# Zhehui-Huang/quad-swarm-rl

Hardware: AMD Instinct MI355X
Metric: env-steps/s (drones x envs x sim_steps) (higher is better)
Workload: dtype f32

## Files before the change

### __graft_entry__.py

```python
import os
import subprocess
import sys

REPO = os.path.dirname(os.path.abspath(__file__))
if REPO not in sys.path:
    sys.path.insert(0, REPO)


def build():
    from quad_swarm_rl_amd import native
    native.build(force=True, verbose=True)
    assert os.path.exists(native.LIB_PATH)
    from quad_swarm_rl_amd import policy
    policy.build(force=True, verbose=True)
    assert os.path.exists(policy.ENC_LIB_PATH)
    subprocess.check_call(["make", "-C", os.path.join(REPO, "oracle"), "-s", "-B"])
    import quad_swarm_rl_amd
    from quad_swarm_rl_amd import config, env
    import ctypes
    lib = ctypes.CDLL(native.LIB_PATH)
    for sym in native.EXPORTED_SYMBOLS + native.EXCHANGE_SYMBOLS:
        getattr(lib, sym)
    paths = prebuild_spec_cache()
    print(f"build ok: {native.LIB_PATH} + {len(paths)} config-specialised code objects in spec_cache/")


def _spec_jobs(with_audit=True):
    import bench
    jobs = []
    for wl in bench.WORKLOADS.values():
        for rew_info in (False, True):
            jobs.append((dict(wl["kw"], num_envs=wl["num_envs"], write_rew_info=rew_info), "f32"))
        jobs.append((dict(wl["kw"], num_envs=wl["num_envs"]), "f64"))
        jobs.append((dict(wl["kw"], num_envs=wl["num_envs"], write_rew_info=False), "f32", 0))
        jobs.append((dict(wl["kw"], num_envs=wl["num_envs"], write_rew_info=False, episode_sums=True), "f32"))
        jobs.append((dict(wl["kw"], num_envs=wl["num_envs"], write_rew_info=True, episode_sums=True), "f32"))
        jobs.append((dict(wl["kw"], num_envs=wl["num_envs"], write_rew_info=False, use_downwash=False), "f32"))
        if not wl["kw"].get("use_obstacles"):
            jobs.append((dict(wl["kw"], num_envs=wl["num_envs"], write_rew_info=False, episode_sums=True, quads_mode="mix"), "f32"))
    smoke_kw = dict(num_envs=4, num_agents=8, neighbor_visible_num=6, neighbor_obs_type="pos_vel", use_downwash=True, use_numba=True,
                    collision_falloff_radius=4.0, rew_coeff=dict(quadcol_bin=5.0, quadcol_bin_smooth_max=10.0))
    jobs += [(smoke_kw, "f64"), (smoke_kw, "f32"), (dict(smoke_kw, write_rew_info=False), "f32")]
    try:
        sys.path.insert(0, os.path.join(REPO, "tests"))
        import test_hip_parity as thp
        for kw in thp.CASES.values():
            jobs += [(dict(kw, num_envs=8), "f64"), (dict(kw, num_envs=8), "f32")]
        for name in ("c2_n8_dw", "c3_n8_obst", "c4_n32_svs"):
            jobs += [(dict(thp.CASES[name], num_envs=512, ep_time=0.3), "f32"), (dict(thp.CASES[name], num_envs=40, ep_time=0.5), "f32"),
                     (dict(thp.CASES[name], num_envs=40, ep_time=0.5), "f64")]
        for name, E in (("c2_n8_dw", 1024), ("c3_n8_obst", 1024), ("c4_n32_svs", 512)):
            jobs.append((dict(thp.CASES[name], num_envs=E, ep_time=0.3), "f64"))
        for name in ("c2_n8_dw", "c4_n32_svs"):
            jobs.append((dict(thp.CASES[name], num_envs=96, ep_time=0.3), "f32"))
        for name in thp.SINGLE_WAVE_CASES:
            jobs += [(dict(thp.CASES[name], num_envs=8), "f64", 0), (dict(thp.CASES[name], num_envs=8), "f32", 0)]
        import test_object_identity_gpu as toi
        for name in toi.POISON_CASES:
            for team in (0, 1):
                kw = dict(thp.CASES[name], num_envs=7, **toi.POISON_OVERRIDES.get(name, {}))
                prec = "f32" if team and kw["num_agents"] > 8 else "f64"
                jobs.append((kw, prec, team))
                jobs += [(kw, prec, team, {"QS_SPEC_EXTRA_FLAGS": f"-DQS_POISON_IDLE={m}"}) for m in (1, 2)]
        for name in toi.SCHED_SINGLE:
            jobs += [(dict(thp.CASES[name], num_envs=7), "f32", 0), (dict(thp.CASES[name], num_envs=7), "f32", 0, {"QS_SPEC_SINGLE_FLAGS": "-mllvm -amdgpu-use-amdgpu-trackers"})]
        for name in ("c2_n8_dw", "c3_n8_obst", "c4_n32_svs"):
            jobs += [(dict(thp.CASES[name], num_envs=7), "f32", 1), (dict(thp.CASES[name], num_envs=7), "f32", 1, {"QS_SPEC_TEAM_FLAGS": ""})]
        for name in toi.RESPONSE_CASES:
            for prec in ("f64", "f32"):
                if prec == "f64" and thp.CASES[name]["num_agents"] > 8:
                    continue
                jobs += [(dict(thp.CASES[name], num_envs=7), prec, 1), (dict(thp.CASES[name], num_envs=7), prec, 1, {"QS_SPEC_EXTRA_FLAGS": "-DQS_SERIAL_PAIR_RESPONSES"})]
        for name in toi.SELECT_CASES:
            jobs += [(dict(thp.CASES[name], num_envs=7), "f32", 0)] + [(dict(thp.CASES[name], num_envs=7), "f32", 0, {"QS_SPEC_EXTRA_FLAGS": f})
                                                                       for f in ("-DQS_EXACT_NBR_SELECT", "-DQS_NBR_TRUNC_BITS=16")]
        for name in toi.STASH_CASES:
            jobs += [(dict(thp.CASES[name], num_envs=7), "f32", 1), (dict(thp.CASES[name], num_envs=7), "f32", 1, {"QS_SPEC_EXTRA_FLAGS": "-DQS_SN_STASH=0"})]
        for name in toi.REDO_CASES:
            jobs += [(dict(thp.CASES[name], num_envs=7), "f32", 1), (dict(thp.CASES[name], num_envs=7), "f32", 1, {"QS_SPEC_EXTRA_FLAGS": "-DQS_REDO_ROWS=0"})]
        import xchg_worker as xw
        jobs += [(dict(xw.KW, num_envs=8, write_rew_info=False), "f32"), (dict(xw.KW, num_envs=4, episode_sums=True), "f32"),
                 (dict(xw.REPLAY_KW, num_envs=8, write_rew_info=False, episode_sums=True), "f32")]
        import test_pilot_gpu as tpg
        jobs.append((dict(tpg.LOOP_KW, num_envs=1024), "f32"))
    except Exception as exc:
        print("spec prebuild: parity cases skipped:", exc)
    finally:
        sys.path.pop(0)
    if with_audit:
        jobs += _audit_jobs()
    return jobs


def _audit_jobs():
    import base64
    import ctypes
    import json
    from quad_swarm_rl_amd import config as qcfg
    path = os.path.join(REPO, "tests", "spec_audit.json")
    if not os.path.exists(path):
        return []
    doc = json.load(open(path))
    if doc.get("sizeof_qs_config") != ctypes.sizeof(qcfg.QsConfig):
        print("spec prebuild: tests/spec_audit.json was written for another qs_config layout - rerun tools/spec_audit.py; skipped")
        return []
    return [(base64.b64decode(o["config"]), None, o["team"]) for o in doc["objects"]]


def _spec_one(job):
    from quad_swarm_rl_amd import config as qcfg, native
    kw, precision = job[0], job[1]
    team = job[2] if len(job) > 2 else -1
    build_env = job[3] if len(job) > 3 else {}
    saved = {k: os.environ.get(k) for k in build_env}
    os.environ.update(build_env)
    try:
        cfg = qcfg.QsConfig.from_buffer_copy(kw) if isinstance(kw, bytes) else qcfg.make_config(precision=precision, **kw)
        return native.spec_build(cfg, team)
    except native.QsError as exc:
        print("spec prebuild skipped:", exc)
        return None
    finally:
        for k, v in saved.items():
            if v is None:
                os.environ.pop(k, None)
            else:
                os.environ[k] = v


def prebuild_spec_cache():
    from concurrent.futures import ProcessPoolExecutor
    jobs = _spec_jobs()
    with ProcessPoolExecutor(max_workers=min(8, os.cpu_count() or 1)) as ex:
        paths = sorted(set(p for p in ex.map(_spec_one, jobs) if p))
    if not paths:
        return paths
    keep = {os.path.splitext(os.path.basename(p))[0] for p in paths}
    cache = os.path.dirname(paths[0])
    for f in os.listdir(cache):
        if os.path.splitext(f)[0] not in keep:
            os.remove(os.path.join(cache, f))
    return paths


def smoke():
    import numpy as np
    from oracle import oracle as orc
    from quad_swarm_rl_amd import config as qcfg, native

    def worst(got, ref, tol, omega_cols=False, relative=False):
        allowed = np.full(ref.shape, tol)
        if relative:
            allowed = tol * np.maximum(1.0, np.abs(ref))
        elif omega_cols:
            allowed[..., 15:18] = tol * np.maximum(1.0, np.abs(ref[..., 15:18]))
        return float((np.abs(got - ref) / allowed).max())

    E, N = 4, 8
    for precision, tol in (("f64", 1e-8), ("f32", 1e-5)):
        cfg = qcfg.make_config(num_envs=E, num_agents=N, neighbor_visible_num=6, neighbor_obs_type="pos_vel",
                               use_downwash=True, use_numba=True, collision_falloff_radius=4.0, seed=11, precision=precision,
                               rew_coeff=dict(quadcol_bin=5.0, quadcol_bin_smooth_max=10.0))
        hip = native.Stepper(cfg, device=0)
        oenvs = [orc.OracleEnv(cfg, env_global_id=e) for e in range(E)]
        oobs = np.stack([o.reset() for o in oenvs])
        hip.reset()
        hobs = hip.to_host("obs").reshape(E, N, -1)
        assert worst(hobs, oobs, tol, omega_cols=True) <= 1.0, (precision, "reset", worst(hobs, oobs, tol, omega_cols=True))
        rng = np.random.RandomState(0)
        for t in range(3):
            act = rng.uniform(-1, 1, size=(E, N, 4)).astype(np.float32).astype(np.float64)
            o = [oe.step(act[e]) for e, oe in enumerate(oenvs)]
            hip.from_host("actions", act.reshape(-1, 4))
            hip.step()
            hip.sync()
            hobs = hip.to_host("obs").reshape(E, N, -1)
            hrew = hip.to_host("reward").reshape(E, N)
            err = max(worst(hobs, np.stack([x[0] for x in o]), tol, omega_cols=True), worst(hrew, np.stack([x[1] for x in o]), tol, relative=True))
            assert err <= 1.0, (precision, t, err)
        hip.check_errors()
        hip.close()
        print(f"smoke {precision}: ok (every observation column within {tol} absolute; angular velocity and reward within {tol} * max(1, |x|))")


if __name__ == "__main__":
    build()
    if len(sys.argv) > 1 and sys.argv[1] == "smoke":
        smoke()
```

### quad-swarm-rl_amd/csrc/qs_nbr_obs.h

```cpp
#pragma once
#include "qs_device.h"

using namespace qs;

__device__ __forceinline__ unsigned long long nbr_key(float m, int idx) {
    const uint32_t b = __float_as_uint(m), o = b ^ ((b >> 31) ? 0xffffffffu : 0x80000000u);
    return ((unsigned long long)o << 32) | (uint32_t)idx;
}

template <typename real> __device__ __forceinline__ real nbr_metric(const real rp[3], const real rv[3]) {
    const real rd = M<real>::fmax(norm3<real>(rp), (real)0.01);
    return rd + (rp[0] * rv[0] + rp[1] * rv[1] + rp[2] * rv[2]) * M<real>::rcp(rd);
}
template <> __device__ __forceinline__ float nbr_metric<float>(const float rp[3], const float rv[3]) {
    const float d2 = __builtin_fmaf(rp[2], rp[2], __builtin_fmaf(rp[1], rp[1], rp[0] * rp[0]));
    const float dot = __builtin_fmaf(rp[2], rv[2], __builtin_fmaf(rp[1], rv[1], rp[0] * rv[0]));
    const float rd = fmaxf(__builtin_amdgcn_sqrtf(d2), 0.01f);
    return __builtin_fmaf(dot, __builtin_amdgcn_rcpf(rd), rd);
}
typedef float qs_f32x2 __attribute__((ext_vector_type(2)));
__device__ __forceinline__ qs_f32x2 nbr_metric_x2(const qs_f32x2 rp[3], const qs_f32x2 rv[3]) {
    const qs_f32x2 d2 = __builtin_elementwise_fma(rp[2], rp[2], __builtin_elementwise_fma(rp[1], rp[1], rp[0] * rp[0]));
    const qs_f32x2 dot = __builtin_elementwise_fma(rp[2], rv[2], __builtin_elementwise_fma(rp[1], rv[1], rp[0] * rv[0]));
    const qs_f32x2 rd = {fmaxf(__builtin_amdgcn_sqrtf(d2.x), 0.01f), fmaxf(__builtin_amdgcn_sqrtf(d2.y), 0.01f)};
    const qs_f32x2 rc = {__builtin_amdgcn_rcpf(rd.x), __builtin_amdgcn_rcpf(rd.y)};
    return __builtin_elementwise_fma(dot, rc, rd);
}
template <typename real> struct NbrKey;
template <> struct NbrKey<float> {
    unsigned long long k;
    static __device__ __forceinline__ NbrKey make(float m, int j) { return {nbr_key(m, j)}; }
    __device__ __forceinline__ bool less(const NbrKey &o) const { return k < o.k; }
    __device__ __forceinline__ int idx() const { return (int)(uint32_t)k; }
    static __device__ __forceinline__ void st(unsigned char *base, int slots, int slot, int B, int tid,
        const NbrKey &v) { ((unsigned long long *)base)[slot * B + tid] = v.k; }
    static __device__ __forceinline__ NbrKey ld(const unsigned char *base, int slots, int slot, int B,
        int tid) { return {((const unsigned long long *)base)[slot * B + tid]}; }
};
template <> struct NbrKey<double> {
    double m; int j;
    static __device__ __forceinline__ NbrKey make(double m, int j) { return {m, j}; }
    __device__ __forceinline__ bool less(const NbrKey &o) const { return (m < o.m) | ((m == o.m) & (j < o.j)); }
    __device__ __forceinline__ int idx() const { return j; }
    static __device__ __forceinline__ void st(unsigned char *base, int slots, int slot, int B, int tid, const NbrKey &v) {
        ((double *)base)[slot * B + tid] = v.m; ((int *)(base + (size_t)slots * B * 8))[slot * B + tid] = v.j; }
    static __device__ __forceinline__ NbrKey ld(const unsigned char *base, int slots, int slot, int B, int tid) {
        return {((const double *)base)[slot * B + tid], ((const int *)(base + (size_t)slots * B * 8))[slot * B + tid]}; }
};

template <typename real>
__device__ __forceinline__ void neighbor_obs(const Consts<real> &c, int N, int i, int base, int B, int tid, const real *s_pos,
    const real *s_vel,
                                             real *s_metric, const real mypos[3], const real myvel[3], real *o) {
    const int K = c.num_neighbors;
    if (K <= 0) return;
    if (K == N - 1 || N <= 8) {
        const bool all_others = (K == N - 1);
        for (int j0 = 0; j0 < N; j0 += 8) {
            real rp[8][3], rv[8][3];
            int rank[8];
#pragma unroll
            for (int u = 0; u < 8; ++u) {
                const int j = (j0 + u < N) ? j0 + u : N - 1;
#pragma unroll
                for (int a = 0; a < 3; ++a) { rp[u][a] = s_pos[a * B + base + j] - mypos[a];
                    rv[u][a] = s_vel[a * B + base + j] - myvel[a]; }
            }
            if (all_others) {
#pragma unroll
                for (int u = 0; u < 8; ++u) rank[u] = (j0 + u < i) ? j0 + u : j0 + u - 1;
            } else {
                real mj[8];
#pragma unroll
                for (int u = 0; u < 8; ++u) {
                    real rd = M<real>::fmax(norm3<real>(rp[u]), (real)0.01);
                    real m = rd + (rp[u][0] * rv[u][0] + rp[u][1] * rv[u][1] + rp[u][2] * rv[u][2]) * M<real>::rcp(rd);
                    mj[u] = (u < N && u != i) ? m : (real)3.4e38;
                    rank[u] = 0;
                }
#pragma unroll
                for (int k = 0; k < 8; ++k)
#pragma unroll
                    for (int u = 0; u < 8; ++u) rank[u] += (int)((mj[k] < mj[u]) | ((mj[k] == mj[u]) & (k < u)));
            }
#pragma unroll
            for (int u = 0; u < 8; ++u) {
                const int j = j0 + u;
                if (j < N && j != i && rank[u] < K) {
                    real *oo = o + rank[u] * 6;
#pragma unroll
                    for (int a = 0; a < 3; ++a) {
                        oo[a] = clipr<real>(rp[u][a], -c.nbr_clip_pos[a], c.nbr_clip_pos[a]);
                        oo[3 + a] = clipr<real>(rv[u][a], -c.nbr_clip_vel[a], c.nbr_clip_vel[a]);
                    }
                }
            }
        }
        return;
    }
    if (K <= 8) {
        real bm[8];
        int bi[8];
#pragma unroll
        for (int k = 0; k < 8; ++k) { bm[k] = (real)3.4e38; bi[k] = 0; }
        for (int j0 = 0; j0 < N; j0 += 4) {
            real rp[4][3], rv[4][3];
#pragma unroll
            for (int u = 0; u < 4; ++u) {
                const int j = (j0 + u < N) ? j0 + u : N - 1;
#pragma unroll
                for (int a = 0; a < 3; ++a) { rp[u][a] = s_pos[a * B + base + j] - mypos[a];
                    rv[u][a] = s_vel[a * B + base + j] - myvel[a]; }
            }
#pragma unroll
            for (int u = 0; u < 4; ++u) {
                const int j = j0 + u;
                real rd = M<real>::fmax(norm3<real>(rp[u]), (real)0.01);
                real m = rd + (rp[u][0] * rv[u][0] + rp[u][1] * rv[u][1] + rp[u][2] * rv[u][2]) * M<real>::rcp(rd);
                m = (j < N && j != i) ? m : (real)3.4e38;
                int mi = j;
#pragma unroll
                for (int k = 0; k < 8; ++k) {
                    const bool lt = m < bm[k];
                    const real tm = lt ? bm[k] : m;
                    const int ti = lt ? bi[k] : mi;
                    bm[k] = lt ? m : bm[k];
                    bi[k] = lt ? mi : bi[k];
                    m = tm; mi = ti;
                }
            }
        }
        real vals[8][6];
#pragma unroll
        for (int k = 0; k < 8; ++k) {
            if (k < K) {
#pragma unroll
                for (int a = 0; a < 3; ++a) { vals[k][a] = s_pos[a * B + base + bi[k]] - mypos[a];
                    vals[k][3 + a] = s_vel[a * B + base + bi[k]] - myvel[a]; }
            }
        }
#pragma unroll
        for (int k = 0; k < 8; ++k) {
            if (k < K) {
#pragma unroll
                for (int a = 0; a < 3; ++a) {
                    o[k * 6 + a] = clipr<real>(vals[k][a], -c.nbr_clip_pos[a], c.nbr_clip_pos[a]);
                    o[k * 6 + 3 + a] = clipr<real>(vals[k][3 + a], -c.nbr_clip_vel[a], c.nbr_clip_vel[a]);
                }
            }
        }
        return;
    }
    for (int j = 0; j < N; ++j) {
        real rp[3] = {s_pos[0 * B + base + j] - mypos[0], s_pos[1 * B + base + j] - mypos[1], s_pos[2 * B + base + j] - mypos[2]};
        real rv[3] = {s_vel[0 * B + base + j] - myvel[0], s_vel[1 * B + base + j] - myvel[1], s_vel[2 * B + base + j] - myvel[2]};
        real rd = M<real>::fmax(norm3<real>(rp), (real)0.01);
        real mm = rd + (rp[0] * rv[0] + rp[1] * rv[1] + rp[2] * rv[2]) * M<real>::rcp(rd);
        s_metric[j * B + tid] = (j == i) ? (real)3.4e38 : mm;
    }
    uint64_t taken = 1ull << i;
    for (int k = 0; k < K; ++k) {
        int best = -1;
        real bmin = (real)3.4e38;
        for (int j = 0; j < N; ++j) {
            real mm = s_metric[j * B + tid];
            bool better = !(taken >> j & 1) && (best < 0 || mm < bmin);
            best = better ? j : best;
            bmin = better ? mm : bmin;
        }
        taken |= 1ull << best;
#pragma unroll
        for (int a = 0; a < 3; ++a) {
            o[k * 6 + a] = clipr<real>(s_pos[a * B + base + best] - mypos[a], -c.nbr_clip_pos[a], c.nbr_clip_pos[a]);
            o[k * 6 + 3 + a] = clipr<real>(s_vel[a * B + base + best] - myvel[a], -c.nbr_clip_vel[a], c.nbr_clip_vel[a]);
        }
    }
}

template <typename real> struct NbrSel {
// ... 244 lines not shown
```

### quad-swarm-rl_amd/csrc/qs_step_team.inc

```
#undef e_state_or_e
#if QS_MULTI
#define e_state_or_e e_state
#else
#define e_state_or_e e
#endif
#ifndef QS_GATED
#define QS_GATED 0
#endif
#ifdef QS_SPEC
#if QS_MULTI && QS_GATED
extern "C" __global__ void __launch_bounds__(64 * QS_TW) qs_spec_gated(QS_KARGS, int QS_EPB_ARG, int ksteps) {
#elif QS_MULTI
extern "C" __global__ void __launch_bounds__(64 * QS_TW) qs_spec_rollout(QS_KARGS, int QS_EPB_ARG, int ksteps) {
#else
extern "C" __global__ void __launch_bounds__(64 * QS_TW) qs_spec_step(QS_KARGS, int QS_EPB_ARG) {
    const int t = 0;
#endif
#else
template <typename real>
#if QS_MULTI && QS_GATED && QS_SCEN_FULL
__global__ void __launch_bounds__(64 * QS_TW) qs_gated_team_full(QS_KARGS, int QS_EPB_ARG, int ksteps) {
#elif QS_MULTI && QS_GATED
__global__ void __launch_bounds__(64 * QS_TW) qs_gated_team(QS_KARGS, int QS_EPB_ARG, int ksteps) {
#elif QS_MULTI && QS_SCEN_FULL
__global__ void __launch_bounds__(64 * QS_TW) qs_rollout_team_full(QS_KARGS, int QS_EPB_ARG, int ksteps) {
#elif QS_MULTI
__global__ void __launch_bounds__(64 * QS_TW) qs_rollout_team(QS_KARGS, int QS_EPB_ARG, int ksteps) {
#elif QS_SCEN_FULL
__global__ void __launch_bounds__(64 * QS_TW) qs_step_team_full(QS_KARGS, int QS_EPB_ARG) {
    const int t = 0;
#else
__global__ void __launch_bounds__(64 * QS_TW) qs_step_team(QS_KARGS, int QS_EPB_ARG) {
    const int t = 0;
#endif
#endif
    extern __shared__ __align__(16) unsigned char smem[];
    constexpr int W = QS_TW, WS = QS_TW - 1;
#ifndef QS_PAIR_ONCE
#define QS_PAIR_ONCE 1
#endif
    QS_SPEC_PROLOGUE
    const Consts<real> *cp = &c;
    real rewc[QS_REW_COUNT + 1];
#pragma unroll
    for (int q = 0; q <= QS_REW_COUNT; ++q) rewc[q] = p.rew_rt[q];
#define QS_OBST_SIZE (c.dr_on ? p.obst_size_env[ee] : c.obst_size)
    const int B = QS_WAVE, N = c.num_agents, E = c.num_envs, T = E * N, M_ = c.num_obstacles, K = c.num_neighbors;
    uint64_t *s_mask = (uint64_t *)(smem + L.off_mask);
    uint32_t *s_envflag = (uint32_t *)(smem + L.off_envflag);
    real *s_pos = (real *)(smem + L.off_pos), *s_vel = (real *)(smem + L.off_vel), *s_zax = (real *)(smem + L.off_zax);
    real *s_om = (real *)(smem + L.off_om), *s_goal = (real *)(smem + L.off_goal), *s_obs = (real *)(smem + L.off_obs);
    real *s_obst = (real *)(smem + L.off_obst), *s_metric = (real *)(smem + L.off_metric);
    real *s_rot6 = (real *)(smem + L.off_t_rot), *s_gpub = (real *)(smem + L.off_t_goal), *s_prox = (real *)(smem + L.off_t_prox);
    uint64_t *s_colm = (uint64_t *)(smem + L.off_t_col), *s_dwm = (uint64_t *)(smem + L.off_t_dw),
        *s_nearm = (uint64_t *)(smem + L.off_t_near);
    int *s_ohit = (int *)(smem + L.off_t_ohit);
    real *s_ri = (real *)(smem + L.off_t_ri);
    int *s_redo = (int *)(smem + L.off_t_redo);
    unsigned char *s_topk = smem + L.off_topk;
    const bool pair_once = QS_PAIR_ONCE && N > 8;
#ifndef QS_SN_STASH
#ifdef QS_SPEC
#define QS_SN_STASH 1
#else
#define QS_SN_STASH 0
#endif
#endif
#ifndef QS_REDO_ROWS
#ifdef QS_SPEC
#define QS_REDO_ROWS 1
#else
#define QS_REDO_ROWS 0
#endif
#endif

    QS_POISON_LDS(L.total, 64 * QS_TW);
    const int wv = __builtin_amdgcn_readfirstlane((int)(threadIdx.x >> 6));
    const int tid = threadIdx.x & 63, le = tid / N, i = tid - le * N, e = blockIdx.x * epb + le, base = le * N;
    const bool active = (le < epb) && (e < E);
    const int g = active ? e * N + i : 0, ee = active ? e : 0;
    const uint64_t nmask = (N >= 64) ? ~0ull : ((1ull << N) - 1);
    real *myobs = s_obs + tid * c.obs_dim;
    const __amdgpu_buffer_rsrc_t rs = QS_BUF_RSRC(p);
    QS_ROW(real, pos, rs, p, T, g); QS_ROW(real, vel, rs, p, T, g); QS_ROW(real, rot, rs, p, T, g); QS_ROW(real, omega, rs, p, T, g);
    QS_ROW(real, rot_damp, rs, p, T, g); QS_ROW(real, cmds_damp, rs, p, T, g); QS_ROW(real, ou, rs, p, T, g);
    QS_ROW(real, goal, rs, p, T, g);
    QS_ROW(real, ring, rs, p, T, g); QS_ROW(real, sums, rs, p, T, g); QS_ROW(uint32_t, flags, rs, p, T, g);
    QS_ROW(uint64_t, pair, rs, p, T, g);

    QS_STAMP(0);
    QS_STAMPW(0);
    QS_STAMP_WG(0);
    Drone<real> d;
    real goal[3], act[4], ring[4], sums[3];
    int32_t cnt[QS_CNT_COUNT];
    uint64_t prev_pair = 0;
    int tick_before = 0, svs_period = 0;
#if QS_SCEN_FULL && defined(QS_SPEC_N)
    ScenRegs<real> sreg;
#endif
    uint32_t step_no = 0;
    uint32_t step_raw = 0;
    if (wv <= 1 || (QS_SN_STASH && !QS_MULTI && wv == 2)) step_raw = p.step_ctr[ee];
    if (wv == 0) {
        if (b_pos.wide) {
            b_pos.template ldv<3>(d.pos); b_vel.template ldv<3>(d.vel); b_omega.template ldv<3>(d.omega); b_goal.template ldv<3>(goal);
            b_sums.template ldv<3>(sums);
            b_rot.template ldv<9>(d.rot);
            b_rot_damp.template ldv<4>(d.rot_damp); b_cmds_damp.template ldv<4>(d.cmds_damp); b_ou.template ldv<4>(d.ou);
            b_ring.template ldv<4>(ring);
        } else {
#pragma unroll
            for (int q = 0; q < 3; ++q) { d.pos[q] = b_pos.ld(q); d.vel[q] = b_vel.ld(q); d.omega[q] = b_omega.ld(q);
                goal[q] = b_goal.ld(q); sums[q] = b_sums.ld(q); }
#pragma unroll
            for (int q = 0; q < 9; ++q) d.rot[q] = b_rot.ld(q);
#pragma unroll
            for (int q = 0; q < 4; ++q) { d.rot_damp[q] = b_rot_damp.ld(q); d.cmds_damp[q] = b_cmds_damp.ld(q); d.ou[q] = b_ou.ld(q);
                ring[q] = b_ring.ld(q); }
        }
        d.flags = b_flags.ld();
        prev_pair = b_pair.ld();
        QS_POISON_DRONE(d); QS_POISON_ARR(goal, 3, 16); QS_POISON_ARR(sums, 3, 16); QS_POISON_ARR(ring, 4, 16); QS_POISON_U64(prev_pair);
        tick_before = p.tick[ee];
        svs_period = (c.scenario == QS_SCENARIO_SWARM_VS_SWARM) ? p.scen_int[ee] : 0;
        if (active && i == 0) {
#pragma unroll
            for (int q = 0; q < QS_CNT_COUNT; ++q) cnt[q] = p.counters[q * E + ee];
        }
#if QS_SCEN_FULL
#ifdef QS_SPEC_N
        if (active) scen_regs_load<real>(p, E, e, i, sreg);
#else
        if (active) scen_lds_load<real>(p, L, smem, E, e, le, i, N);
#endif
#endif
        asm volatile("" : "+v"(step_raw));
        step_no = step_raw + 1;
    } else if (wv == 1 || (QS_SN_STASH && !QS_MULTI && wv == 2)) {
        step_no = step_raw + 1;
    }
    if (wv == W - 1 && c.use_obstacles && active) {
        for (int k = i; k < M_; k += N) {
            s_obst[(le * 2 + 0) * M_ + k] = p.obst_pos[(size_t)e * M_ + k];
            s_obst[(le * 2 + 1) * M_ + k] = p.obst_pos[(size_t)E * M_ + (size_t)e * M_ + k];
        }
    }
#if QS_SCEN_FULL
    real *s_sr = (real *)(smem + L.off_sr) + le * SR_COUNT;
    int *s_si = (int *)(smem + L.off_si) + le * SI_COUNT;
#endif
    constexpr int WL = 2;
    const bool logw = (wv == WL) && active;
    real rsum[QS_SUM_COUNT];
    if (logw && c.episode_sums) {
#pragma unroll
        for (int q = 0; q < QS_SUM_COUNT; ++q) rsum[q] = p.run_sums[q * T + g];
    }
#if !QS_MULTI
    unsigned long long xq_seq = 0, xq_ack = ~0ull;
    if constexpr (sizeof(real) == 4) {
        if (p.xchg != nullptr) {
            xq_seq = p.xchg->loc->push_seq;
            if (wv == 0 && tid < p.xchg->world) xq_ack = qsx::ld_sys(&p.xchg->mine->ack[tid]);
        }
    }
#endif
    uint64_t out_curr_pair = 0;
    bool nan_any = false;
#if QS_MULTI
    const int g_state = g, e_state = e;
#if QS_GATED
    qsx::Gate *const G = (qsx::Gate *)p.xchg;
    const unsigned long long gseq0 = (unsigned long long)(uintptr_t)actions;
    bool gate_dead = false;
    unsigned long long *s_pre_seq = (unsigned long long *)s_ri;
    unsigned int *s_actpre = (unsigned int *)((char *)s_ri + 16);
    unsigned long long pf_flag = 0, pf_flag_next = 0;
    if (threadIdx.x == 0) *s_pre_seq = 0;
#endif
    for (int t = 0; t < ksteps; ++t) {
    int g = g_state, e = e_state;
    asm volatile("" : "+v"(g), "+v"(e));
#endif
    RngKey key = {c.seed_lo, c.seed_hi, (uint32_t)(c.env_id_offset + ee), step_no};
    SensNoise<real> sn;
    real rew = 0, ri[QS_RI_COUNT];
    bool nan_rew = false, done = false;
    int tick = 0;
#if QS_GATED
    bool pf_hold_issue = false;
    unsigned int pf_hold[sizeof(real)] = {};
#endif
    if (wv == 0) {
#if QS_GATED
        {
            const unsigned long long seq = gseq0 + (unsigned long long)t + 1;
            if (*s_pre_seq == seq) {
                if constexpr (sizeof(real) == 4) {
#pragma unroll
                    for (int q = 0; q < 4; ++q) act[q] = __uint_as_float(s_actpre[tid * 4 + q]);
                } else {
#pragma unroll
                    for (int q = 0; q < 4; ++q) act[q] = __longlong_as_double(((long long)s_actpre[tid * 8 + 2 * q + 1] << 32) | s_actpre[tid * 8 + 2 * q]);
                }
            } else {
            if (!gate_dead && !qsx::poll_ge_agent(&G->act_flag[blockIdx.x / G->wg_per_group], seq, G->timeout_ticks)) {
                gate_dead = true;
                if (tid == 0) atomicOr(&G->status, 1u);
            }
            const char *a = G->act_ring + ((seq - 1) % G->ring_len) * G->act_stride + (size_t)g * 4 * sizeof(real);
            if constexpr (sizeof(real) == 4) {
                const qsx::u32x4_t v = qsx::ld16_sc1(a);
                act[0] = __uint_as_float(v.x); act[1] = __uint_as_float(v.y); act[2] = __uint_as_float(v.z); act[3] = __uint_as_float(v.w);
            } else {
                const qsx::u32x4_t v0 = qsx::ld16_sc1(a), v1 = qsx::ld16_sc1(a + 16);
                act[0] = __longlong_as_double(((long long)v0.y << 32) | v0.x);
                act[1] = __longlong_as_double(((long long)v0.w << 32) | v0.z);
                act[2] = __longlong_as_double(((long long)v1.y << 32) | v1.x);
                act[3] = __longlong_as_double(((long long)v1.w << 32) | v1.z);
            }
            }
        }
#else
        {
            const real *a = actions + ((size_t)t * T + g) * 4;
#pragma unroll
// ... 150 lines not shown
    if (wv == 1) {
        QS_SELF_OBS_W1();
    } else if (active) {
        const int lane3 = (wv == 0) ? 0 : wv - 1;
        const real mp[3] = {s_pos[0 * B + tid], s_pos[1 * B + tid], s_pos[2 * B + tid]};
        const real pr = rewc[QS_REW_COUNT];
        uint32_t colm_lo = 0, colm_hi = 0, dwm_lo = 0, dwm_hi = 0;
        real prox = 0;
        for (int j0 = lane3; j0 < N; j0 += 2 * WS) {
            real rel[2][3], zx[2][3];
#pragma unroll
            for (int u = 0; u < 2; ++u) {
                const int j = (j0 + WS * u < N) ? j0 + WS * u : N - 1;
#pragma unroll
                for (int a = 0; a < 3; ++a) { rel[u][a] = mp[a] - s_pos[a * B + base + j]; zx[u][a] = s_zax[a * B + base + j]; }
            }
#pragma unroll
            for (int u = 0; u < 2; ++u) {
                const int j = j0 + WS * u;
                const bool other = (j < N) & (j != i);
                real dist = M<real>::sqrt(rel[u][0] * rel[u][0] + rel[u][1] * rel[u][1] + rel[u][2] * rel[u][2]);
                const uint32_t hit = (uint32_t)(other & (dist <= c.collision_threshold));
                prox += (other & (dist <= c.collision_falloff_threshold)) ? pr * dist + rewc[QS_REW_QUADCOL_SMOOTH_MAX] : (real)0;
                real rz = dot3<real>(rel[u], zx[u]), rxy = M<real>::sqrt(dist * dist - rz * rz);
                const uint32_t dw = (uint32_t)(other & ((real)-0.7 < rz) & (rz < (real)0) & (rxy < (real)0.1));
                if (N <= 32 || j < 32) { colm_lo |= hit << (j & 31); dwm_lo |= dw << (j & 31); }
                else { colm_hi |= hit << (j & 31); dwm_hi |= dw << (j & 31); }
            }
        }
        const uint64_t colm = colm_lo | ((uint64_t)colm_hi << 32), dwm = dwm_lo | ((uint64_t)dwm_hi << 32);
        if (colm) atomicOr((unsigned long long *)&s_colm[tid], (unsigned long long)colm);
        if (dwm) atomicOr((unsigned long long *)&s_dwm[tid], (unsigned long long)dwm);
        s_prox[lane3 * B + tid] = prox;
        if (wv == W - 1) {
            int obst_idx = -1;
            if (c.use_obstacles) {
                const real *ox = s_obst + (le * 2 + 0) * M_, *oy = s_obst + (le * 2 + 1) * M_;
                for (int k = M_ - 1; k >= 0; --k) {
                    real dx = mp[0] - ox[k], dy = mp[1] - oy[k];
                    obst_idx = (M<real>::sqrt(dx * dx + dy * dy) <= (c.dr_on
                        ? c.arm_r + (real)0.5 * QS_OBST_SIZE : c.obst_hit_threshold)) ? k : obst_idx;
                }
            }
            s_ohit[tid] = obst_idx;
        }
    }
    QS_STAMPW(3);
    QS_TEAM_BARRIER();
    QS_STAMP(6); QS_STAMP_WGK(8);
    QS_STAMPW(4);

    uint64_t curr_pair = 0, unique = 0, m_obst_new = 0, m_room = 0, new_pair = 0;
    bool refresh_obs = false;
    int obst_idx = -1;
    real eps_dist[3] = {0, 0, 0};
    if (wv == 0) {
        uint64_t dw_mask = 0;
        bool in_curr = false;
        real prox = 0;
        uint32_t bits = 0;
        if (active) {
            const uint64_t colm = s_colm[tid];
            in_curr = colm != 0;
            curr_pair = (i >= 63) ? 0 : (colm & ~((2ull << i) - 1));
            dw_mask = s_dwm[tid];
            if (pair_once) {
                uint64_t nm = s_nearm[tid];
                while (__builtin_expect(nm != 0, 0)) {
                    const int j = __ffsll((long long)nm) - 1;
                    nm &= nm - 1;
                    const real rel[3] = {d.pos[0] - s_pos[0 * B + base + j], d.pos[1] - s_pos[1 * B + base + j],
                        d.pos[2] - s_pos[2 * B + base + j]};
                    prox += rewc[QS_REW_COUNT] * M<real>::sqrt(rel[0] * rel[0] + rel[1] * rel[1] + rel[2] * rel[2]) + rewc[QS_REW_QUADCOL_SMOOTH_MAX];
                }
            } else {
                prox = s_prox[0 * B + tid];
#pragma unroll
                for (int q = 1; q < WS; ++q) prox += s_prox[q * B + tid];
            }
            if (c.use_obstacles) {
                obst_idx = s_ohit[tid];
                obstacle_hit_bits(obst_idx, d.flags, bits);
            }
            room_collision_bits(d.flags, bits);
        }
        new_pair = curr_pair & ~prev_pair;
        const EnvEvents ev = env_events<real>(c, active, in_curr, new_pair, bits, d.flags, base, nmask, i, tick, tick_before, myobs);
        unique = ev.unique; m_obst_new = ev.obst_new; m_room = ev.room;
        collision_rewards<real>(c, rewc, ev, i, bits, prox, rew, ri);
        if (c.write_rew_info || c.episode_sums) {
#pragma unroll
            for (int q = 0; q < QS_RI_COUNT; ++q) s_ri[q * B + tid] = ri[q];
            s_ri[QS_RI_COUNT * B + tid] = done ? (real)1 : (real)0;
        }
#if QS_SCEN_FULL
        goal_distance_log<real, false>(c, active ? s_sr[SR_METRIC] : (real)0, tick, done, d.flags, ring, sums, ri, eps_dist);
#else
        goal_distance_log<real, false>(c, c.approach_goal_metric, tick, done, d.flags, ring, sums, ri, eps_dist);
#endif
        if (active && i == 0) env_counters_add<real>(c, cnt, ev);

        QS_STAMP(7); QS_STAMP_WGK(9);
        const real vel_before[3] = {d.vel[0], d.vel[1], d.vel[2]};
        downwash_phase<real>(c, key, d, s_pos, s_zax, B, base, nmask, N, i, active, dw_mask, bits, (int *)nullptr,
            (const double *)nullptr, WaveSync());
        QS_STAMP(8);
        const bool any_dw = ((__ballot(active && (bits & B_DOWNWASH)) >> base) & nmask) != 0;
        static_assert((W - 1) * QS_WAVE >= QS_DD_CHUNK * QS_DD_DRAWS, "the draw table fits the proximity rows");
#ifdef QS_SERIAL_PAIR_RESPONSES
        pair_responses<real>(key, d, ev, new_pair, active, N, i, tid, base, B, s_pos, s_vel, s_om, s_mask, (int *)nullptr, WaveSync());
#else
        pair_responses<real>(key, d, ev, new_pair, active, N, i, tid, base, B, s_pos, s_vel, s_om, s_mask, (int *)nullptr, WaveSync(), s_prox);
#endif
        room_obstacle_phase<real>(cp, key, d, active, N, i, bits, obst_idx, s_obst + (le * 2 + 0) * M_, s_obst + (le * 2 + 1) * M_,
            p.obst_size_env + ee, (int *)nullptr, WaveSync());
        const bool update_flag = any_dw || (ev.newpair_any != 0) || (ev.obst_new != 0) || (ev.wall != 0) || (ev.ceil != 0);

#if QS_SCEN_FULL
        {
            ScenCtx<real> x = {s_sr, s_si, (uint64_t *)(smem + L.off_omap) + le * 4, s_goal + le * L.goal_rows * 3, s_zax, B, base, N};
            scenario_phase_full<real>(c, key, x, active, N, i, tick, goal, (int *)s_mask + base, (int *)nullptr, WaveSync());
        }
#else
        svs_phase<real>(c, p, key, active, N, E, e, i, tick, svs_period, s_goal + le * L.goal_rows * 3, (int *)s_mask + base, goal,
            (int *)nullptr, WaveSync());
#endif
        QS_STAMP(9); QS_STAMP_WGK(10);
#pragma unroll
        for (int q = 0; q < 3; ++q) s_vel[q * B + tid] = d.vel[q];
        refresh_obs = update_flag && active;
        if (pair_once) {
            const bool vel_changed = active && (bits_differ(d.vel[0], vel_before[0]) | bits_differ(d.vel[1], vel_before[1]) |
                bits_differ(d.vel[2], vel_before[2]));
            const uint32_t changed = (uint32_t)((__ballot(vel_changed) >> base) & nmask);
            if (active && i == 0) s_redo[le] = QS_REDO_ROWS && N <= 32 ? (int)changed : (update_flag ? 1 : 0);
        } else if (__builtin_expect(refresh_obs, 0)) {
            if (c.sense_noise) {
                if (stash_sn) {
                    const real *o = myobs + c.self_dim;
#pragma unroll
                    for (int q = 0; q < 3; ++q) { sn.p[q] = o[q]; sn.v[q] = o[3 + q]; sn.w[q] = o[6 + q]; sn.th[q] = o[9 + q]; }
                } else sensor_noise_draw<real>(c, key, i, 1, sn);
            }
            self_obs<real>(c, sn, d, goal, myobs);
        }
    } else if (pair_once) {
        if (wv == 1 && !c.use_obstacles) QS_SELF_OBS_W1();
        if (ranked && K <= 8 && active) team_rank_local<real, W>(N, i, base, B, tid, wv, s_pos, s_vel, s_metric, s_topk, false);
    }
    QS_STAMPW(5);
    QS_TEAM_BARRIER();
    QS_STAMP(14); QS_STAMP_WGK(11);
    QS_STAMPW(6);
    real mpos[3] = {0, 0, 0}, mvel[3] = {0, 0, 0};
    if (K > 0 && active) {
#pragma unroll
        for (int q = 0; q < 3; ++q) { mpos[q] = s_pos[q * B + tid]; mvel[q] = s_vel[q * B + tid]; }
    }
    const bool po_big = pair_once && K > 0 && K < N - 1 && K <= 8;
    const bool redo = pair_once && active && s_redo[le] != 0;
    if (QS_REDO_ROWS && N <= 32 && po_big) {
        bool wg_redo = false;
        for (int q = 0; q < epb; ++q) wg_redo |= s_redo[q] != 0;
        if (__builtin_expect(wg_redo, 0)) {
            if (wv >= 1) {
                uint32_t m = active ? (uint32_t)s_redo[le] : 0u;
                for (int idx = 0; __any(m != 0); ++idx) {
                    const int a = m ? __ffs((int)m) - 1 : -1;
                    m &= m - 1;
                    if (a >= 0 && a != i && idx % (W - 1) == wv - 1) {
                        const real rp[3] = {s_pos[0 * B + base + a] - mpos[0], s_pos[1 * B + base + a] - mpos[1], s_pos[2 * B + base + a] - mpos[2]};
                        const real rv[3] = {s_vel[0 * B + base + a] - mvel[0], s_vel[1 * B + base + a] - mvel[1], s_vel[2 * B + base + a] - mvel[2]};
                        const real mm = nbr_metric<real>(rp, rv);
                        s_metric[a * B + tid] = mm; s_metric[i * B + base + a] = mm;
                    }
                }
            }
            QS_TEAM_BARRIER();
            if (wv >= 1 && redo) team_rank_local<real, W>(N, i, base, B, tid, wv, s_pos, s_vel, s_metric, s_topk, false);
        }
    }
    if (pair_once && wv == 0 && __builtin_expect(refresh_obs, 0)) {
        if (c.sense_noise) {
            if (stash_sn) {
                const real *o = myobs + c.self_dim;
#pragma unroll
                for (int q = 0; q < 3; ++q) { sn.p[q] = o[q]; sn.v[q] = o[3 + q]; sn.w[q] = o[6 + q]; sn.th[q] = o[9 + q]; }
            } else sensor_noise_draw<real>(c, key, i, 1, sn);
        }
        self_obs<real>(c, sn, d, goal, myobs);
    }
    if (logw && (c.write_rew_info || c.episode_sums)) {
        real r[QS_RI_COUNT];
#pragma unroll
        for (int q = 0; q < QS_RI_COUNT; ++q) r[q] = s_ri[q * B + tid];
        const bool fin = s_ri[QS_RI_COUNT * B + tid] != (real)0;
        if (c.write_rew_info) {
#pragma unroll
            for (int q = 0; q < QS_RI_COUNT; ++q) p.rew_info[q * T + g] = r[q];
        }
        if (c.episode_sums) {
            real a4[4];
#if QS_GATED
            {
                const char *a = G->act_ring + ((gseq0 + (unsigned long long)t) % G->ring_len) * G->act_stride + (size_t)g * 4 * sizeof(real);
#pragma unroll
                for (int q = 0; q < 4; ++q) {
                    if constexpr (sizeof(real) == 4) a4[q] = __uint_as_float(qsx::ld4_sc1(a + 4 * q));
                    else a4[q] = __longlong_as_double(((long long)qsx::ld4_sc1(a + 8 * q + 4) << 32) | qsx::ld4_sc1(a + 8 * q));
                }
            }
#else
            {
                const real *a = actions + ((size_t)t * T + g) * 4;
#pragma unroll
                for (int q = 0; q < 4; ++q) a4[q] = a[q];
            }
#endif
#pragma unroll
            for (int q = 0; q < QS_SUM_COUNT; ++q) {
                const real add = q < QS_RI_COUNT
                    ? r[q < QS_RI_COUNT ? q : 0] : (q < QS_SUM_ACT2
                    ? a4[(q - QS_SUM_ACT) & 3] : a4[(q - QS_SUM_ACT2) & 3] * a4[(q - QS_SUM_ACT2) & 3]);
                const real v = rsum[q] + add;
                if (fin) p.ep_sums[q * T + g] = v;
                rsum[q] = fin ? (real)0 : v;
            }
        }
    }
#ifdef QS_EXP_NOBIG
    const bool big = false;
#else
    const bool big = !pair_once && N > 8 && K <= 8;
#endif
    real bm[8];
    int bi[8];
    int *s_mlist_i = (int *)(s_metric + W * 8 * B);
    if (QS_REDO_ROWS && N <= 32 && po_big) {
    } else
    if (po_big && wv >= 1 && __builtin_expect(redo, 0)) team_rank_local<real,
        W>(N, i, base, B, tid, wv, s_pos, s_vel, s_metric, s_topk, true);
    if (ranked && active && !big && !po_big && (!pair_once || redo)) {
        for (int j0 = wv; j0 < N; j0 += 2 * W) {
            real rp[2][3], rv[2][3];
#pragma unroll
            for (int u = 0; u < 2; ++u) {
                const int j = (j0 + W * u < N) ? j0 + W * u : N - 1;
#pragma unroll
                for (int a = 0; a < 3; ++a) { rp[u][a] = s_pos[a * B + base + j] - mpos[a]; rv[u][a] = s_vel[a * B + base + j] - mvel[a]; }
            }
#pragma unroll
            for (int u = 0; u < 2; ++u) {
                const int j = j0 + W * u;
                real rd = M<real>::fmax(norm3<real>(rp[u]), (real)0.01);
                real m = rd + (rp[u][0] * rv[u][0] + rp[u][1] * rv[u][1] + rp[u][2] * rv[u][2]) * M<real>::rcp(rd);
                if (j < N) s_metric[j * B + tid] = (j != i) ? m : (real)3.4e38;
            }
        }
    }
    if (ranked && active && big) {
#pragma unroll
        for (int k = 0; k < 8; ++k) { bm[k] = (real)3.4e38; bi[k] = 0x7fffffff; }
        for (int j0 = wv; j0 < N; j0 += 2 * W) {
            real rp[2][3], rv[2][3];
#pragma unroll
            for (int u = 0; u < 2; ++u) {
                const int j = (j0 + W * u < N) ? j0 + W * u : N - 1;
#pragma unroll
                for (int a = 0; a < 3; ++a) { rp[u][a] = s_pos[a * B + base + j] - mpos[a]; rv[u][a] = s_vel[a * B + base + j] - mvel[a]; }
            }
#pragma unroll
            for (int u = 0; u < 2; ++u) {
                const int j = j0 + W * u;
                real rd = M<real>::fmax(norm3<real>(rp[u]), (real)0.01);
                real m = rd + (rp[u][0] * rv[u][0] + rp[u][1] * rv[u][1] + rp[u][2] * rv[u][2]) * M<real>::rcp(rd);
                const bool valid = (j < N) & (j != i);
                m = valid ? m : (real)3.4e38;
                int mi = valid ? j : 0x7fffffff;
#pragma unroll
                for (int k = 0; k < 8; ++k) {
                    const bool lt = m < bm[k];
                    const real tm = lt ? bm[k] : m;
                    const int ti = lt ? bi[k] : mi;
                    bm[k] = lt ? m : bm[k];
                    bi[k] = lt ? mi : bi[k];
                    m = tm; mi = ti;
                }
            }
        }
        if constexpr (sizeof(real) == 4) {
            unsigned long long *s_keys = (unsigned long long *)s_metric;
#pragma unroll
            for (int k = 0; k < 8; ++k) s_keys[(wv * 8 + k) * B + tid] = nbr_key((float)bm[k], bi[k]);
        } else {
#pragma unroll
            for (int k = 0; k < 8; ++k) { s_metric[(wv * 8 + k) * B + tid] = bm[k]; s_mlist_i[(wv * 8 + k) * B + tid] = bi[k]; }
        }
    }
    QS_STAMPW(7);
    QS_TEAM_BARRIER();
    QS_STAMP(15); QS_STAMP_WGK(12);
    QS_STAMPW(8);
    if (po_big && active && wv >= 1) {
        constexpr int SL = (W - 1) * 8;
        NbrKey<real> own[8];
        int grank[8];
#pragma unroll
        for (int r = 0; r < 8; ++r) { if (r < K) own[r] = NbrKey<real>::ld(s_topk, SL, (wv - 1) * 8 + r, B, tid); grank[r] = r; }
        for (int w2 = 1; w2 < W; ++w2) {
            if (w2 == wv) continue;
            NbrKey<real> ok[8];
#pragma unroll
            for (int q = 0; q < 8; ++q) if (q < K) ok[q] = NbrKey<real>::ld(s_topk, SL, (w2 - 1) * 8 + q, B, tid);
#pragma unroll
            for (int r = 0; r < 8; ++r) {
                if (r < K) {
#pragma unroll
                    for (int q = 0; q < 8; ++q) if (q < K) grank[r] += (int)ok[q].less(own[r]);
                }
            }
        }
        real *o = myobs + c.self_dim;
#pragma unroll
        for (int r = 0; r < 8; ++r) {
            if (r < K) {
                const int j = own[r].idx();
                if (j < N && grank[r] < K) {
                    real *oo = o + grank[r] * 6;
                    real vals[6];
#pragma unroll
                    for (int a = 0; a < 3; ++a) { vals[a] = s_pos[a * B + base + j]; vals[3 + a] = s_vel[a * B + base + j]; }
#pragma unroll
                    for (int a = 0; a < 3; ++a) {
                        oo[a] = clipr<real>(vals[a] - mpos[a], -c.nbr_clip_pos[a], c.nbr_clip_pos[a]);
                        oo[3 + a] = clipr<real>(vals[3 + a] - mvel[a], -c.nbr_clip_vel[a], c.nbr_clip_vel[a]);
                    }
                }
            }
        }
    }
    if (K > 0 && active && !(ranked && (big || po_big))) {
        real *o = myobs + c.self_dim;
        for (int j = wv; j < N; j += W) {
            if (j == i) continue;
            int rank = (j < i) ? j : j - 1;
            if (ranked) {
                const real mj = s_metric[j * B + tid];
                rank = 0;
                for (int k0 = 0; k0 < N; k0 += 8) {
                    real mk[8];
#pragma unroll
                    for (int u = 0; u < 8; ++u) mk[u] = s_metric[((k0 + u < N) ? k0 + u : N - 1) * B + tid];
#pragma unroll
                    for (int u = 0; u < 8; ++u) rank += (int)((k0 + u < N) & ((mk[u] < mj) | ((mk[u] == mj) & (k0 + u < j))));
                }
            }
            if (rank < K) {
                real *oo = o + rank * 6;
                real vals[6];
#pragma unroll
                for (int a = 0; a < 3; ++a) { vals[a] = s_pos[a * B + base + j]; vals[3 + a] = s_vel[a * B + base + j]; }
#pragma unroll
                for (int a = 0; a < 3; ++a) {
                    oo[a] = clipr<real>(vals[a] - mpos[a], -c.nbr_clip_pos[a], c.nbr_clip_pos[a]);
                    oo[3 + a] = clipr<real>(vals[3 + a] - mvel[a], -c.nbr_clip_vel[a], c.nbr_clip_vel[a]);
                }
            }
        }
    }
    if (ranked && big && active) {
        real *o = myobs + c.self_dim;
        int grank[8];
#pragma unroll
        for (int k = 0; k < 8; ++k) grank[k] = k;
        if constexpr (sizeof(real) == 4) {
            const unsigned long long *s_keys = (const unsigned long long *)s_metric;
            unsigned long long mk[8];
#pragma unroll
            for (int k = 0; k < 8; ++k) mk[k] = nbr_key((float)bm[k], bi[k]);
            for (int w2 = 0; w2 < W; ++w2) {
                if (w2 == wv) continue;
                unsigned long long ok[8];
#pragma unroll
                for (int q = 0; q < 8; ++q) ok[q] = s_keys[(w2 * 8 + q) * B + tid];
#pragma unroll
                for (int k = 0; k < 8; ++k) {
                    if (k < K) {
#pragma unroll
                        for (int q = 0; q < 8; ++q) grank[k] += (int)(ok[q] < mk[k]);
                    }
                }
            }
        } else {
            for (int w2 = 0; w2 < W; ++w2) {
                if (w2 == wv) continue;
                real om[8];
                int oi[8];
#pragma unroll
                for (int q = 0; q < 8; ++q) { om[q] = s_metric[(w2 * 8 + q) * B + tid]; oi[q] = s_mlist_i[(w2 * 8 + q) * B + tid]; }
#pragma unroll
                for (int k = 0; k < 8; ++k)
#pragma unroll
                    for (int q = 0; q < 8; ++q) grank[k] += (int)((om[q] < bm[k]) | ((om[q] == bm[k]) & (oi[q] < bi[k])));
            }
        }
#pragma unroll
        for (int k = 0; k < 8; ++k) {
            if (k < K && bi[k] < N && grank[k] < K) {
                const int j = bi[k];
                real *oo = o + grank[k] * 6;
                real vals[6];
#pragma unroll
                for (int a = 0; a < 3; ++a) { vals[a] = s_pos[a * B + base + j]; vals[3 + a] = s_vel[a * B + base + j]; }
#pragma unroll
                for (int a = 0; a < 3; ++a) {
                    oo[a] = clipr<real>(vals[a] - mpos[a], -c.nbr_clip_pos[a], c.nbr_clip_pos[a]);
                    oo[3 + a] = clipr<real>(vals[3 + a] - mvel[a], -c.nbr_clip_vel[a], c.nbr_clip_vel[a]);
                }
            }
        }
    }
    if (c.use_obstacles && active) {
        const real *ox = s_obst + (le * 2 + 0) * M_, *oy = s_obst + (le * 2 + 1) * M_;
        const real px = s_pos[0 * B + tid], py = s_pos[1 * B + tid];
        real *o = myobs + c.self_dim + 6 * K;
        for (int q = wv; q < 9; q += W) {
            const int a = q / 3, b = q - a * 3;
            const real gx = px + (real)0.1 * (real)(a - 1), gy = py + (real)0.1 * (real)(b - 1);
            real mind2 = (real)10000;
            for (int k = 0; k < M_; ++k) {
                real dx = gx - ox[k], dy = gy - oy[k], d2 = dx * dx + dy * dy;
                mind2 = d2 < mind2 ? d2 : mind2;
            }
            o[q] = M<real>::sqrt(mind2) - (c.dr_on ? (real)0.5 * QS_OBST_SIZE : c.obst_radius);
        }
    }
    QS_STAMPW(9);
    QS_TEAM_BARRIER();
    QS_STAMP(10); QS_STAMP_WGK(13);
    QS_STAMPW(10);

    uint64_t out_unique = unique, out_obst_new = m_obst_new, out_room = m_room, out_new_pair = new_pair;
    out_curr_pair = curr_pair;
    int out_tick = tick, out_obst_idx = obst_idx;
    if (wv == 0) {
        const bool do_reset = active && done;
        if (__builtin_expect(__ballot(do_reset) != 0, 0)) {
            if (do_reset) {
                p.ep_stats[QS_EPS_DIST_1S * T + g] = eps_dist[0]; p.ep_stats[QS_EPS_DIST_3S * T + g] = eps_dist[1];
                p.ep_stats[QS_EPS_DIST_5S * T + g] = eps_dist[2];
                p.ep_stats[QS_EPS_REACHED_GOAL * T + g] = (d.flags & F_REACHED) ? (real)1 : (real)0;
                p.ep_stats[QS_EPS_COL_AGENT_OK * T + g] = (d.flags & F_COL_AGENT_OK) ? (real)1 : (real)0;
                p.ep_stats[QS_EPS_COL_OBST_OK * T + g] = (d.flags & F_COL_OBST_OK) ? (real)1 : (real)0;
                if (i == 0) {
#pragma unroll
                    for (int q = 0; q < QS_CNT_COUNT; ++q) { p.ep_counters[q * E + e] = cnt[q]; cnt[q] = 0; }
                }
            }
            real stale_vel[3] = {d.vel[0], d.vel[1], d.vel[2]};
            QS_WAVE_SYNC();
            if (do_reset && i == 0) p.ep_scenario[e] = QS_SCEN_FULL ? ((int *)(smem + L.off_si))[le * SI_COUNT + SI_SCEN] : c.scenario;
            reset_body<real, (QS_SCEN_FULL != 0), true>(cp, &p, &L, smem, epb, key, do_reset, &d, goal, stale_vel);
            if (do_reset) {
                out_unique = 0; out_obst_new = 0; out_room = 0; out_curr_pair = 0; out_new_pair = 0; out_tick = 0; out_obst_idx = -1;
                ring[0] = ring[1] = ring[2] = ring[3] = 0;
                if (c.scenario == QS_SCENARIO_SWARM_VS_SWARM) svs_period = (int)s_envflag[epb + le];
            }
        }
    }
    QS_STAMP(11); QS_STAMP_WGK(14);
    QS_STAMPW(11);
    QS_TEAM_BARRIER();
    QS_STAMPW(12);
    {
        const int D = c.obs_dim, first_env = blockIdx.x * epb;
        int nenv = E - first_env; nenv = nenv < epb ? nenv : epb;
        const int total = nenv * N * D;
        real *dst = p.obs + (size_t)first_env * N * D;
#if QS_GATED
        {
            if ((total & 3) == 0 && ((((size_t)first_env * N * D) * sizeof(real)) & 15) == 0 && sizeof(real) == 4) {
                const qsx::u32x4_t *src4 = (const qsx::u32x4_t *)s_obs;
                for (int idx = threadIdx.x; idx < total / 4; idx += 64 * W) qsx::st16_sc1((float *)dst + 4 * idx, src4[idx]);
            } else if constexpr (sizeof(real) == 4) {
                for (int idx = threadIdx.x; idx < total; idx += 64 * W) qsx::st4_sc1(dst + idx, __float_as_uint((float)s_obs[idx]));
            } else {
                for (int idx = threadIdx.x; idx < total; idx += 64 * W) qsx::st8_sc1(dst + idx,
                    (unsigned long long)__double_as_longlong((double)s_obs[idx]));
            }
        }
#else
        if ((total & 3) == 0 && ((((size_t)first_env * N * D) * sizeof(real)) & 15) == 0 && sizeof(real) == 4) {
            const qs_f32x4 *src4 = (const qs_f32x4 *)s_obs;
            for (int idx = threadIdx.x; idx < total / 4; idx += 64 * W) obs_st4((float *)dst + 4 * idx, src4[idx]);
// ... 222 lines not shown
```

Before: 2.344 billion.

## Compute small-team neighbor ranks per row in 8-lane groups via DPP

For teams of 8 waves with at most 8 agents, each thread now takes one (agent, neighbor) pair and computes the metric. Ranks within each 8-lane row come from DPP lane shuffles instead of writing metrics to LDS, waiting at a team barrier, and having each agent loop over all others. This removes the metric LDS round-trip, the barrier, and the serial per-agent rank loop. The cost is a different thread-to-work mapping that depends on W==8 and N<=8, which is enabled by default only in spec builds.

```diff
diff --git a/__graft_entry__.py b/__graft_entry__.py
--- a/__graft_entry__.py
+++ b/__graft_entry__.py
@@ -78,6 +78,10 @@
             jobs += [(dict(thp.CASES[name], num_envs=7), "f32", 1), (dict(thp.CASES[name], num_envs=7), "f32", 1, {"QS_SPEC_EXTRA_FLAGS": "-DQS_SN_STASH=0"})]
         for name in toi.REDO_CASES:
             jobs += [(dict(thp.CASES[name], num_envs=7), "f32", 1), (dict(thp.CASES[name], num_envs=7), "f32", 1, {"QS_SPEC_EXTRA_FLAGS": "-DQS_REDO_ROWS=0"})]
+        import test_team_tail_identity_gpu as ttt
+        for name, prec in ttt.RUNS:
+            jobs += [(dict(thp.CASES[name], num_envs=7), prec, 1)] + [(dict(thp.CASES[name], num_envs=7), prec, 1, {"QS_SPEC_EXTRA_FLAGS": f"-D{sw}=0"})
+                                                                      for sw in ttt.SWITCHES]
         import xchg_worker as xw
         jobs += [(dict(xw.KW, num_envs=8, write_rew_info=False), "f32"), (dict(xw.KW, num_envs=4, episode_sums=True), "f32"),
                  (dict(xw.REPLAY_KW, num_envs=8, write_rew_info=False, episode_sums=True), "f32")]
diff --git a/quad-swarm-rl_amd/csrc/qs_nbr_obs.h b/quad-swarm-rl_amd/csrc/qs_nbr_obs.h
--- a/quad-swarm-rl_amd/csrc/qs_nbr_obs.h
+++ b/quad-swarm-rl_amd/csrc/qs_nbr_obs.h
@@ -25,6 +25,27 @@
     const qs_f32x2 rd = {fmaxf(__builtin_amdgcn_sqrtf(d2.x), 0.01f), fmaxf(__builtin_amdgcn_sqrtf(d2.y), 0.01f)};
     const qs_f32x2 rc = {__builtin_amdgcn_rcpf(rd.x), __builtin_amdgcn_rcpf(rd.y)};
     return __builtin_elementwise_fma(dot, rc, rd);
+}
+template <int CTRL> __device__ __forceinline__ float qs_dpp_mov(float x) {
+    return __int_as_float(__builtin_amdgcn_update_dpp(0, __float_as_int(x), CTRL, 0xf, 0xf, false));
+}
+template <int CTRL> __device__ __forceinline__ double qs_dpp_mov(double x) {
+    const int lo = __builtin_amdgcn_update_dpp(0, __double2loint(x), CTRL, 0xf, 0xf, false);
+    const int hi = __builtin_amdgcn_update_dpp(0, __double2hiint(x), CTRL, 0xf, 0xf, false);
+    return __hiloint2double(hi, lo);
+}
+template <typename real> __device__ __forceinline__ int nbr_rank_group8(real m, int j, int N) {
+    constexpr int QX1 = 0xB1, QX2 = 0x4E, QX3 = 0x1B, HALF_MIRROR = 0x141;
+    const real h = qs_dpp_mov<HALF_MIRROR>(m);
+    const real mk[7] = {qs_dpp_mov<QX1>(m), qs_dpp_mov<QX2>(m), qs_dpp_mov<QX3>(m), qs_dpp_mov<QX3>(h), qs_dpp_mov<QX2>(h),
+        qs_dpp_mov<QX1>(h), h};
+    int rank = 0;
+#pragma unroll
+    for (int x = 1; x < 8; ++x) {
+        const int k = j ^ x;
+        rank += (int)((k < N) & ((mk[x - 1] < m) | ((mk[x - 1] == m) & (k < j))));
+    }
+    return rank;
 }
 template <typename real> struct NbrKey;
 template <> struct NbrKey<float> {
diff --git a/quad-swarm-rl_amd/csrc/qs_step_team.inc b/quad-swarm-rl_amd/csrc/qs_step_team.inc
--- a/quad-swarm-rl_amd/csrc/qs_step_team.inc
+++ b/quad-swarm-rl_amd/csrc/qs_step_team.inc
@@ -73,6 +73,14 @@
 #define QS_REDO_ROWS 0
 #endif
 #endif
+#ifndef QS_NBR_ROWLANES
+#ifdef QS_SPEC
+#define QS_NBR_ROWLANES 1
+#else
+#define QS_NBR_ROWLANES 0
+#endif
+#endif
+    const bool rowlanes = QS_NBR_ROWLANES && W == 8 && N <= 8;
 
     QS_POISON_LDS(L.total, 64 * QS_TW);
     const int wv = __builtin_amdgcn_readfirstlane((int)(threadIdx.x >> 6));
@@ -529,8 +537,30 @@
     QS_TEAM_BARRIER();
     QS_STAMP(14); QS_STAMP_WGK(11);
     QS_STAMPW(6);
+    if (rowlanes && K > 0) {
+        const int rt = (int)(threadIdx.x >> 3), rj = (int)(threadIdx.x & 7), rle = rt / N, ri = rt - rle * N;
+        const bool rvalid = (rle < epb) & ((int)blockIdx.x * epb + rle < E) & (rj < N) & (rj != ri);
+        const int pj = rvalid ? rle * N + rj : rt;
+        real rp[3], rv[3];
+#pragma unroll
+        for (int a = 0; a < 3; ++a) { rp[a] = s_pos[a * B + pj] - s_pos[a * B + rt]; rv[a] = s_vel[a * B + pj] - s_vel[a * B + rt]; }
+        int rank = (rj < ri) ? rj : rj - 1;
+        if (ranked) {
+            real rd = M<real>::fmax(norm3<real>(rp), (real)0.01);
+            real m = rd + (rp[0] * rv[0] + rp[1] * rv[1] + rp[2] * rv[2]) * M<real>::rcp(rd);
+            rank = nbr_rank_group8<real>(rvalid ? m : (real)3.4e38, rj, N);
+        }
+        if (rvalid && rank < K) {
+            real *oo = s_obs + rt * c.obs_dim + c.self_dim + rank * 6;
+#pragma unroll
+            for (int a = 0; a < 3; ++a) {
+                oo[a] = clipr<real>(rp[a], -c.nbr_clip_pos[a], c.nbr_clip_pos[a]);
+                oo[3 + a] = clipr<real>(rv[a], -c.nbr_clip_vel[a], c.nbr_clip_vel[a]);
+            }
+        }
+    }
     real mpos[3] = {0, 0, 0}, mvel[3] = {0, 0, 0};
-    if (K > 0 && active) {
+    if (K > 0 && active && !rowlanes) {
 #pragma unroll
         for (int q = 0; q < 3; ++q) { mpos[q] = s_pos[q * B + tid]; mvel[q] = s_vel[q * B + tid]; }
     }
@@ -617,7 +647,7 @@
     } else
     if (po_big && wv >= 1 && __builtin_expect(redo, 0)) team_rank_local<real,
         W>(N, i, base, B, tid, wv, s_pos, s_vel, s_metric, s_topk, true);
-    if (ranked && active && !big && !po_big && (!pair_once || redo)) {
+    if (ranked && active && !big && !po_big && !rowlanes && (!pair_once || redo)) {
         for (int j0 = wv; j0 < N; j0 += 2 * W) {
             real rp[2][3], rv[2][3];
 #pragma unroll
@@ -675,7 +705,7 @@
         }
     }
     QS_STAMPW(7);
-    QS_TEAM_BARRIER();
+    if (!rowlanes) QS_TEAM_BARRIER();
     QS_STAMP(15); QS_STAMP_WGK(12);
     QS_STAMPW(8);
     if (po_big && active && wv >= 1) {
@@ -716,7 +746,7 @@
             }
         }
     }
-    if (K > 0 && active && !(ranked && (big || po_big))) {
+    if (K > 0 && active && !rowlanes && !(ranked && (big || po_big))) {
         real *o = myobs + c.self_dim;
         for (int j = wv; j < N; j += W) {
             if (j == i) continue;
```

Result: faster. 2.409 billion, median of 6 (+2.8%).
